# ClarkMcGrew/root-simple-mcmc

Measured on AMD Instinct MI355X. Metric: chain-steps/s on D=50 TDummyLogLikelihood, 65 536 chains; ESS/s + accept rate, higher is better.
Workload: dtype f64

## Files before the change

root-simple-mcmc_amd/csrc/smcmc_host.hpp:

```cpp
#pragma once

#include <hip/hip_runtime.h>

#include <cstddef>
#include <string>
#include <vector>

#include "smcmc.h"
#include "smcmc_event_sample_host.hpp"
#include "smcmc_kernels.hip.h"

namespace smcmc {

template <typename T, bool Pinned = false>
class Buffer {
public:
    Buffer() = default;
    ~Buffer() { release(); }
    Buffer(Buffer&& o) noexcept : p_(o.p_), n_(o.n_) { o.p_ = nullptr; o.n_ = 0; }
    Buffer& operator=(Buffer&& o) noexcept {
        if (this != &o) {
            release();
            p_ = o.p_; n_ = o.n_;
            o.p_ = nullptr; o.n_ = 0;
        }
        return *this;
    }
    Buffer(const Buffer&) = delete;
    Buffer& operator=(const Buffer&) = delete;

    hipError_t allocate(size_t n) {
        release();
        void* p = nullptr;
        const hipError_t e = Pinned ? hipHostMalloc(&p, n * sizeof(T), hipHostMallocDefault) : hipMalloc(&p, n * sizeof(T));
        if (e != hipSuccess) return e;
        p_ = static_cast<T*>(p);
        n_ = n;
        return hipSuccess;
    }
    size_t size() const { return n_; }
    T* get() const { return p_; }
    operator T*() const { return p_; }

private:
    void release() {
        if (p_) (void)(Pinned ? hipHostFree(p_) : hipFree(p_));
        p_ = nullptr;
        n_ = 0;
    }
    T* p_ = nullptr;
    size_t n_ = 0;
};
template <typename T> using DeviceBuffer = Buffer<T, false>;
template <typename T> using PinnedBuffer = Buffer<T, true>;

struct DeviceGuard {
    int prev = -1;
    bool switched = false;
    explicit DeviceGuard(int device) {
        if (hipGetDevice(&prev) == hipSuccess && prev != device) switched = (hipSetDevice(device) == hipSuccess);
    }
    ~DeviceGuard() {
        if (switched) (void)hipSetDevice(prev);
    }
    DeviceGuard(const DeviceGuard&) = delete;
    DeviceGuard& operator=(const DeviceGuard&) = delete;
};
#define ON_DEVICE(h) ::smcmc::DeviceGuard device_guard_((h)->device)

template <typename H>
int fail(H* h, int status, const std::string& msg) {
    if (h) h->error = msg;
    return status;
}

#define HIP_TRY(h, expr)                                                                                  \
    do {                                                                                                  \
        hipError_t e_ = (expr);                                                                           \
        if (e_ != hipSuccess)                                                                             \
            return ::smcmc::fail((h), SMCMC_ERR_HIP, std::string(#expr) + ": " + hipGetErrorString(e_)); \
    } while (0)

#define SMCMC_DP_ENTRY(n) n,
constexpr int kDPList[] = {SMCMC_FOR_EACH_DP(SMCMC_DP_ENTRY)};
#undef SMCMC_DP_ENTRY
constexpr int kNumDP = sizeof(kDPList) / sizeof(kDPList[0]);

inline bool event_likelihood(int like) {
    return like == SMCMC_LIKE_EVENT_SAMPLE || like == SMCMC_LIKE_EVENT_TEMPLATE || like == SMCMC_LIKE_EVENT_SHAPE;
}
inline int event_likelihood_dim(int like) { return like == SMCMC_LIKE_EVENT_SHAPE ? SMCMC_ESH_DIM : SMCMC_ES_DIM; }

inline bool stress_likelihood(int like) {
    return like == SMCMC_LIKE_ASYM || like == SMCMC_LIKE_HORRIFIC || like == SMCMC_LIKE_CONSTRAINED;
}

inline int pick_dp(int dim, int like) {
    for (int i = 0; i < kNumDP; ++i)
        if (dim <= kDPList[i] && (!stress_likelihood(like) || kDPList[i] == 31 || kDPList[i] == 63)) return kDPList[i];
    return -1;
}

template <typename T>
__global__ void fill_kernel(T* dst, size_t n, T v) {
    const size_t i = (size_t)blockIdx.x * blockDim.x + threadIdx.x;
    if (i < n) dst[i] = v;
}

template <typename T>
hipError_t fill(T* dst, size_t n, T v, hipStream_t stream) {
    const int threads = 256;
    hipLaunchKernelGGL(HIP_KERNEL_NAME(fill_kernel<T>), dim3((unsigned)((n + threads - 1) / threads)), dim3(threads), 0,
                       stream, dst, n, v);
    return hipGetLastError();
}

template <typename H>
int check_like_params(H* h, int like, size_t user_max, const char* user_rule, std::vector<double>& prm) {
    const std::vector<double>& p = h->like_params;
    prm.clear();
    switch (like) {
        case SMCMC_LIKE_QUADFORM:
            if (p.size() != (size_t)h->dim * h->dim)
                return fail(h, SMCMC_ERR_INVALID, "QUADFORM needs dim*dim likelihood parameters (the Error matrix)");
            break;
        case SMCMC_LIKE_ROSENBROCK:
            prm = {p.empty() ? 100.0 : p[0]};
            break;
        case SMCMC_LIKE_ASYM:
            if (p.empty()) prm = {-1.0, 100.0};
            else if (p.size() == 2) prm = p;
            else return fail(h, SMCMC_ERR_INVALID, "ASYM takes {positiveSlope, negativeSlope}");
            break;
        case SMCMC_LIKE_CONSTRAINED:
            if (p.size() != 2 + 2 * (size_t)h->dim)
                return fail(h, SMCMC_ERR_INVALID,
                            "CONSTRAINED needs {SummedValues, SummedConstraint, ExpectedValues[dim], PriorConstraints[dim]}");
            prm = p;
            break;
        case SMCMC_LIKE_EVENT_SAMPLE:
        case SMCMC_LIKE_EVENT_TEMPLATE:
        case SMCMC_LIKE_EVENT_SHAPE: {
            const char* why = es_check_like(like, p.data(), p.size());
            if (why) return fail(h, SMCMC_ERR_INVALID, why);
            break;
        }
        case SMCMC_LIKE_USER:
            if (p.size() > user_max) return fail(h, SMCMC_ERR_INVALID, user_rule);
            prm = p;
            break;
        default: break;
    }
    return SMCMC_OK;
}

// ... 2 lines not shown
```

root-simple-mcmc_amd/csrc/smcmc_inst.hip:

```cpp
#include "smcmc_kernels.hip.h"
#include "smcmc_vaat_kernel.hip.h"

#if !defined(SMCMC_DP) || !defined(SMCMC_LIKE)
#error "compile with -DSMCMC_DP=<padded dimension> -DSMCMC_LIKE=<likelihood id>"
#endif

namespace smcmc {

template <int DP, int LIKE, bool EXACT, bool FULLU, bool MOM, bool SPECIAL>
static hipError_t go(const StepParams& p, hipStream_t s) {
    if constexpr (LIKE == SMCMC_LIKE_EVENT_SAMPLE || LIKE == SMCMC_LIKE_EVENT_TEMPLATE || LIKE == SMCMC_LIKE_EVENT_SHAPE) {
        auto kernel = step_kernel<DP, LIKE, EXACT, FULLU, MOM, SPECIAL>;
        constexpr int cap = event_lds_bytes(LIKE, event_max_bins(LIKE));
        if (p.like_lds_bytes <= 0 || p.like_lds_bytes > cap) return hipErrorInvalidValue;
        if (LIKE != SMCMC_LIKE_EVENT_SAMPLE && !p.like_park) return hipErrorInvalidValue;
        const hipError_t e = hipFuncSetAttribute(reinterpret_cast<const void*>(kernel), hipFuncAttributeMaxDynamicSharedMemorySize, cap);
        if (e != hipSuccess) return e;
        hipLaunchKernelGGL(kernel, dim3(p.npad / kWave), dim3(kWave), (size_t)p.like_lds_bytes, s, p);
        return hipGetLastError();
    }
    hipLaunchKernelGGL(HIP_KERNEL_NAME(step_kernel<DP, LIKE, EXACT, FULLU, MOM, SPECIAL>), dim3(p.npad / kWave),
                       dim3(kWave), 0, s, p);
    return hipGetLastError();
}

template <>
hipError_t launch_step_like<SMCMC_DP, SMCMC_LIKE>(const StepParams& p, bool exact, bool fullu, bool mom, bool special,
                                                  hipStream_t s) {
    constexpr int DP = SMCMC_DP, LIKE = SMCMC_LIKE;
#if SMCMC_LIKE == 7 || SMCMC_LIKE == 8 || SMCMC_LIKE == 9
    if (!exact) return hipErrorNotSupported;
    if (special) {
        if (fullu) return mom ? go<DP, LIKE, true, true, true, true>(p, s) : go<DP, LIKE, true, true, false, true>(p, s);
        return mom ? go<DP, LIKE, true, false, true, true>(p, s) : go<DP, LIKE, true, false, false, true>(p, s);
    }
    if (fullu) return mom ? go<DP, LIKE, true, true, true, false>(p, s) : go<DP, LIKE, true, true, false, false>(p, s);
    return mom ? go<DP, LIKE, true, false, true, false>(p, s) : go<DP, LIKE, true, false, false, false>(p, s);
#else
    if (special) {
        if (!exact) return hipErrorNotSupported;
        if (fullu) return mom ? go<DP, LIKE, true, true, true, true>(p, s) : go<DP, LIKE, true, true, false, true>(p, s);
        return mom ? go<DP, LIKE, true, false, true, true>(p, s) : go<DP, LIKE, true, false, false, true>(p, s);
    }
    if (fullu) return mom ? go<DP, LIKE, true, true, true, false>(p, s) : go<DP, LIKE, true, true, false, false>(p, s);
    if (exact) return mom ? go<DP, LIKE, true, false, true, false>(p, s) : go<DP, LIKE, true, false, false, false>(p, s);
    return mom ? go<DP, LIKE, false, false, true, false>(p, s) : go<DP, LIKE, false, false, false, false>(p, s);
#endif
}

#if (SMCMC_LIKE != 3 || defined(SMCMC_USER_LIKELIHOOD)) && SMCMC_LIKE != 7 && SMCMC_LIKE != 8 && SMCMC_LIKE != 9
template <>
hipError_t launch_vaat_like<SMCMC_DP, SMCMC_LIKE>(const VaatParams& p, bool exact, hipStream_t s) {
    constexpr int DP = SMCMC_DP, LIKE = SMCMC_LIKE;
    if (p.record != nullptr) {
        if (exact) hipLaunchKernelGGL(HIP_KERNEL_NAME(vaat_step_kernel<DP, LIKE, true, true>), dim3(p.npad / kWave), dim3(kWave), 0, s, p);
        else hipLaunchKernelGGL(HIP_KERNEL_NAME(vaat_step_kernel<DP, LIKE, false, true>), dim3(p.npad / kWave), dim3(kWave), 0, s, p);
        return hipGetLastError();
    }
    if (exact) hipLaunchKernelGGL(HIP_KERNEL_NAME(vaat_step_kernel<DP, LIKE, true>), dim3(p.npad / kWave), dim3(kWave), 0, s, p);
    else hipLaunchKernelGGL(HIP_KERNEL_NAME(vaat_step_kernel<DP, LIKE, false>), dim3(p.npad / kWave), dim3(kWave), 0, s, p);
    return hipGetLastError();
}
#endif

#if SMCMC_LIKE == 0
template <>
hipError_t launch_reduce<SMCMC_DP>(double* gacc, int ngroups, int D, double* chunk_sums, double* moments,
                                   hipStream_t s) {
    const int npk = (D + 1) * (D + 2) / 2;
    const int nchunks = (ngroups + kReduceChunk - 1) / kReduceChunk;
    hipLaunchKernelGGL(HIP_KERNEL_NAME(reduce_chunks_kernel<SMCMC_DP>), dim3((npk + 63) / 64, nchunks), dim3(64), 0, s,
// ... 10 lines not shown
```

root-simple-mcmc_amd/csrc/smcmc_kernels.hip.h:

```cpp
#pragma once

#include <hip/hip_runtime.h>
#include <stdint.h>

#include <type_traits>

#include "smcmc.h"
#include "smcmc_detmath.h"
#include "smcmc_event_sample.h"
#include "smcmc_step_deal.h"

namespace smcmc {

#define SMCMC_FOR_EACH_DP(X) X(7) X(15) X(31) X(47) X(50) X(63)

#define SMCMC_DP_ENTRY(n) n,
constexpr int kDpMacroList[] = {SMCMC_FOR_EACH_DP(SMCMC_DP_ENTRY)};
#undef SMCMC_DP_ENTRY
constexpr bool dp_lists_agree() {
    if (sizeof(kDpMacroList) / sizeof(kDpMacroList[0]) != (size_t)kNumDpFamilies) return false;
    for (int f = 0; f < kNumDpFamilies; ++f)
        if (kDpMacroList[f] != kDpFamilies[f]) return false;
    return true;
}
static_assert(dp_lists_agree(), "kDpFamilies of smcmc_step_deal.h restates SMCMC_FOR_EACH_DP: keep the two alike");

constexpr int kWave = 64;

typedef double f64x4 __attribute__((ext_vector_type(4)));

typedef const __attribute__((address_space(4))) double* cptr_f64;
typedef const __attribute__((address_space(3))) double* lds_cptr_f64;
typedef double f64x2 __attribute__((ext_vector_type(2)));
typedef const __attribute__((address_space(3))) f64x2* lds_cptr_f64x2;
__device__ __forceinline__ cptr_f64 as_const(const double* p) {
#pragma clang diagnostic push
#pragma clang diagnostic ignored "-Wold-style-cast"
    return (cptr_f64)p;
#pragma clang diagnostic pop
}


struct NormalTables { f64x2 le, ae; };
template <int DP>
constexpr bool kAsmReads = DP >= 47;
template <bool ASM>
__device__ __forceinline__ NormalTables normal_tables_fetch(uint32_t w0, uint32_t w1, uint32_t lt_base, uint32_t at_base) {
    NormalTables t;
    const uint32_t la = lt_base + 16u * smcmc_normal_log_index(w0), aa = at_base + 16u * smcmc_normal_angle_index_halfcircle(w1);
    if constexpr (ASM) {
        asm volatile("ds_read_b128 %0, %1" : "=v"(t.le) : "v"(la));
        asm volatile("ds_read_b128 %0, %1" : "=v"(t.ae) : "v"(aa));
    } else {
        t.le = *(volatile lds_cptr_f64x2)(uintptr_t)la;
        t.ae = *(volatile lds_cptr_f64x2)(uintptr_t)aa;
    }
    return t;
}
template <int N, bool ASM>
__device__ __forceinline__ void normal_tables_ready(NormalTables& a, NormalTables& b) {
    if constexpr (ASM) asm volatile("s_waitcnt lgkmcnt(%4)" : "+v"(a.le), "+v"(a.ae), "+v"(b.le), "+v"(b.ae) : "n"(N));
}
template <int N, bool ASM>
__device__ __forceinline__ void normal_tables_ready(NormalTables& a) {
    if constexpr (ASM) asm volatile("s_waitcnt lgkmcnt(%2)" : "+v"(a.le), "+v"(a.ae) : "n"(N));
}
__device__ __forceinline__ void normal_pair_lds(uint32_t w0, uint32_t w1, const NormalTables& t, double* n0, double* n1) {
#ifdef SMCMC_NORMAL_TEXTBOOK
    (void)t;
    smcmc_normal_pair(w0, w1, n0, n1);
    return;
#endif
#define SMCMC_LT_LDS(k, c) (t.le[c])
#define SMCMC_AT_LDS(c) (t.ae[c])
    SMCMC_NORMAL_PAIR_BODY_HALFCIRCLE(SMCMC_LT_LDS, SMCMC_AT_LDS)
#undef SMCMC_LT_LDS
#undef SMCMC_AT_LDS
}

template <int I, int N, typename F>
__device__ __forceinline__ void static_for_impl(F& f) {
    if constexpr (I < N) {
        f(std::integral_constant<int, I>{});
        static_for_impl<I + 1, N>(f);
    }
}
template <int N, typename F>
__device__ __forceinline__ void static_for(F&& f) { static_for_impl<0, N>(f); }

template <int DP, bool FULLU, int i, int c, int k = 0>
__device__ __forceinline__ void load_piece(uint32_t ubase, f64x2 (&dst)[kPiece / 2]) {
    typedef ULayout<DP, FULLU> UL;
    if constexpr (k < kPiece / 2) {
        if constexpr (c + 2 * k < UL::DPE) {
            constexpr int off = (UL::off(i) + (c - UL::j0(i)) + 2 * k) * 8;
            if constexpr (kAsmReads<DP>) asm volatile("ds_read_b128 %0, %1 offset:%2" : "=v"(dst[k]) : "v"(ubase), "n"(off));
            else dst[k] = *(lds_cptr_f64x2)(uintptr_t)(ubase + (uint32_t)off);
        }
        load_piece<DP, FULLU, i, c, k + 1>(ubase, dst);
    }
}
template <int N, int M, bool ASM>
// ... 414 lines not shown
            const double pj = xq[XL::row(j)];
            if constexpr (EXACT) logl -= h * e * pj;
            else logl = SMCMC_FMA(-(h * e), pj, logl);
        }
    }
    return logl;
}

struct QuadCsr {
    const int32_t* rowptr;
    const int32_t* cols;
    const double* vals;
    const int32_t* rows;
};
constexpr int kQuadChunk = 8;
typedef const __attribute__((address_space(4))) int32_t* cptr_i32;
__device__ __forceinline__ cptr_i32 as_const(const int32_t* p) {
#pragma clang diagnostic push
#pragma clang diagnostic ignored "-Wold-style-cast"
    return (cptr_i32)p;
#pragma clang diagnostic pop
}
template <bool EXACT, typename Point>
__device__ __forceinline__ double quadform_csr(const Point& point, const QuadCsr& q, int D) {
    const cptr_i32 rw = as_const(q.rows), cl = as_const(q.cols);
    const cptr_f64 vl = as_const(q.vals);
    const int nnz = as_const(q.rowptr)[0];
    double logl = 0.0;
    for (int k0 = 0; k0 < nnz; k0 += kQuadChunk) {
        int ri[kQuadChunk], ci[kQuadChunk];
        double e[kQuadChunk], pi[kQuadChunk], pj[kQuadChunk];
#pragma unroll
        for (int u = 0; u < kQuadChunk; ++u) {
            ri[u] = rw[k0 + u];
            ci[u] = cl[k0 + u];
            e[u] = vl[k0 + u];
        }
#pragma unroll
        for (int u = 0; u < kQuadChunk; ++u) {
            pi[u] = point(ri[u]);
            pj[u] = point(ci[u]);
        }
#pragma unroll
        for (int u = 0; u < kQuadChunk; ++u) {
            const double h = 0.5 * pi[u];
            if constexpr (EXACT) logl -= h * e[u] * pj[u];
            else logl = SMCMC_FMA(-(h * e[u]), pj[u], logl);
        }
    }
    (void)D;
    return logl;
}

template <int DP, int LIKE, bool EXACT, bool FULLU, bool MOMENTS, bool SPECIAL>
__global__ void __launch_bounds__(kWave, 2) step_kernel(const StepParams p) {
    constexpr int T = Geo<DP>::T;
    constexpr int NT = Geo<DP>::NT;
    constexpr int NB = Geo<DP>::NB;
    typedef ULayout<DP, FULLU> UL;
    constexpr bool HEADLINE = EXACT && !FULLU && !SPECIAL && DP == 50 && LIKE == SMCMC_LIKE_ISO_GAUSS;
    constexpr bool PAIRS = HEADLINE;
    constexpr bool FIXED_AW = HEADLINE && MOMENTS && AcceptBlock<DP>::FIXED;
    typedef XLayout<DP, MOMENTS, PAIRS> XL;
    static_assert(!PAIRS || DP % 2 == 0, "a lane's 16-byte accesses cover whole row pairs of the point");
    constexpr bool ZROW = HEADLINE && MOMENTS;
    static_assert(!ZROW || XL::ZERO_ROW == DP + 1, "the ones row's partner is the zero row");
    __shared__ alignas(PAIRS ? 16 : 8) double xs[XL::DOUBLES];
    __shared__ __attribute__((aligned(16))) double us[UL::SIZE];
    __shared__ __attribute__((aligned(16))) double ntab[384];

    double* es_hist = nullptr;
    if constexpr (LIKE == SMCMC_LIKE_EVENT_SAMPLE || LIKE == SMCMC_LIKE_EVENT_TEMPLATE || LIKE == SMCMC_LIKE_EVENT_SHAPE) {
        extern __shared__ __attribute__((aligned(16))) double es_dynamic[];
        es_hist = es_dynamic;
    }
    (void)es_hist;

    const int lane = threadIdx.x;
    const int group = blockIdx.x;
    const int chain = group * kWave + lane;
    const bool active = chain < p.nchains;
    const int D = p.dim;
    const size_t NP = (size_t)p.npad;
    const uint32_t gid = p.chain_offset + (uint32_t)chain;
    const cptr_f64 c0 = as_const(p.c0);
    const cptr_f64 likep = as_const(p.like);
    double* const xcol = xs + XL::LANE * lane;
    auto load_point = [&](double (&dst)[DP]) {
#pragma unroll
        for (int q = 0; q < DP / 2; ++q) {
            const f64x2 v = *(const f64x2*)(xcol + XL::row(2 * q));
            dst[2 * q] = v[0];
            dst[2 * q + 1] = v[1];
        }
    };
    auto store_point = [&](const double (&src)[DP]) {
#pragma unroll
        for (int q = 0; q < DP / 2; ++q) {
            f64x2 v;
            v[0] = src[2 * q];
            v[1] = src[2 * q + 1];
            *(f64x2*)(xcol + XL::row(2 * q)) = v;
        }
    };
    (void)load_point;
    (void)store_point;

    if constexpr (PAIRS) {
        double xin[DP];
#pragma unroll
        for (int d = 0; d < DP; ++d) xin[d] = active ? p.x[(size_t)d * NP + chain] : c0[d];
        store_point(xin);
    } else {
#pragma unroll
        for (int d = 0; d < DP; ++d) xcol[XL::row(d)] = active ? p.x[(size_t)d * NP + chain] : c0[d];
    }

    double* lf = p.lane_f64 + chain;
    int32_t* li = p.lane_i32 + chain;
    double logl = lf[SMCMC_LANE_LOGL * NP];
    double sigma = lf[SMCMC_LANE_SIGMA * NP];
    double acc_rate = lf[SMCMC_LANE_ACCEPTANCE * NP];
    double acc_trials = lf[SMCMC_LANE_ACCEPTANCE_TRIALS * NP];
    double rigid = lf[SMCMC_LANE_RIGIDITY * NP];
    double last_value = lf[SMCMC_LANE_LAST_VALUE * NP];
    double last_x0 = lf[SMCMC_LANE_LAST_X0 * NP];
    double step_rms = lf[SMCMC_LANE_STEP_RMS * NP];
    double logl_prop = lf[SMCMC_LANE_LOGL_PROPOSED * NP];
    int trials = li[SMCMC_LANE_TRIALS * NP];
    int succ = li[SMCMC_LANE_SUCCESSES * NP];
    int next_update = li[SMCMC_LANE_NEXT_UPDATE * NP];
    int naccept = li[SMCMC_LANE_NACCEPT * NP];
    int rms_trials = li[SMCMC_LANE_STEP_RMS_TRIALS * NP];
    int last_accept = li[SMCMC_LANE_LAST_ACCEPT * NP];

#pragma unroll
    for (int i = 0; i < DP; ++i) {
        for (int k = lane; k < UL::len(i); k += kWave) {
            const int j = UL::j0(i) + k;
            us[UL::off(i) + k] = (j < DP) ? p.U[i * DP + j] : 0.0;
        }
    }

    for (int k = lane; k < 128; k += kWave) ntab[k] = smcmc_log_table_dev[k];
    for (int k = lane; k < 64; k += kWave) {
        const double c = smcmc_angle_table_dev[2 * k], sn = smcmc_angle_table_dev[2 * k + 1];
        ntab[128 + 2 * k] = c;
        ntab[128 + 2 * k + 1] = sn;
        ntab[128 + 128 + 2 * k] = -sn;
        ntab[128 + 128 + 2 * k + 1] = c;
    }
    const uint32_t ltab = (uint32_t)(uintptr_t)(lds_cptr_f64)ntab, atab = ltab + 128u * 8u;

    constexpr bool STRIP = MOMENTS && Geo<DP>::STRIP;
    constexpr int NT16 = Geo<DP>::NT16;
    f64x4 acc[MOMENTS ? NT16 : 1];
    double accs[STRIP ? T : 1];
    double c0r[MOMENTS ? T : 1];
    int xrow[MOMENTS ? T : 1];
    double c0s = 0.0;
    int xsrow = 0;
    if constexpr (MOMENTS) {
#pragma unroll
        for (int t = 0; t < NT16; ++t)
#pragma unroll
            for (int r = 0; r < 4; ++r)
                acc[t][r] = p.gacc[(((size_t)group * NT + t) * 4 + r) * kWave + lane];
        if constexpr (STRIP) {
#pragma unroll
            for (int t = 0; t < T; ++t) accs[t] = p.gacc[(((size_t)group * NT + NT16 + t) * 4) * kWave + lane];
            const int r = 16 * Geo<DP>::T16 + (lane & 3);
            c0s = (r < DP) ? p.c0[r] : 0.0;
            xsrow = XL::row((r <= DP) ? r : (ZROW ? XL::ZERO_ROW : DP)) + XL::LANE * (lane >> 4);
        }
        if constexpr (PAIRS) {
            static_assert(XL::HELD == DP + 2, "the ones row and its partner are one pair");
            f64x2 ones;
            ones[0] = active ? 1.0 : 0.0;
            ones[1] = 0.0;
            *(f64x2*)(xcol + XL::row(DP)) = ones;
        } else {
            xcol[XL::row(DP)] = active ? 1.0 : 0.0;
        }
#pragma unroll
        for (int t = 0; t < T; ++t) {
            const int r = 16 * t + (lane & 15);
            c0r[t] = (r < DP) ? p.c0[r] : 0.0;
            xrow[t] = XL::row((r <= DP) ? r : (ZROW ? XL::ZERO_ROW : DP)) + XL::LANE * (lane >> 4);
        }
    }
    __syncthreads();

    constexpr bool OPF = MOMENTS && T >= 3 && kAsmReads<DP> && DP <= 50 && !FULLU && !SPECIAL;
    constexpr int KQ = 4 * 8 * XL::LANE;
    double raw[OPF ? T : 1], raws = 0.0;
    uint32_t xaddr[OPF ? T : 1], xsaddr = 0;
    if constexpr (OPF) {
#pragma unroll
        for (int t = 0; t < T; ++t) xaddr[t] = (uint32_t)(uintptr_t)(lds_cptr_f64)(xs + xrow[t]);
        if constexpr (STRIP) xsaddr = (uint32_t)(uintptr_t)(lds_cptr_f64)(xs + xsrow);
    }

    double xp[DP];
    const uint32_t aw = smcmc_accept_word((uint32_t)D);
#ifdef SMCMC_STEP_PROFILE
// ... 70 lines not shown
            if (dense) logl_prop = loglike_quadform_lds<DP, EXACT, XL>(xcol, likep + p.zero * (s + 1));
        }
        else if constexpr (LIKE == SMCMC_LIKE_EVENT_SAMPLE) logl_prop = event_sample_loglike<DP>(xp, likep + p.zero * (s + 1), es_hist, lane);
        else if constexpr (LIKE == SMCMC_LIKE_EVENT_TEMPLATE)
            logl_prop = event_two_pass_loglike<DP, false>(xp, likep + p.zero * (s + 1), es_hist, lane, p.like_park + chain, NP);
        else if constexpr (LIKE == SMCMC_LIKE_EVENT_SHAPE)
            logl_prop = event_two_pass_loglike<DP, true>(xp, likep + p.zero * (s + 1), es_hist, lane, p.like_park + chain, NP);
        else if constexpr (!RMS_AHEAD) logl_prop = loglike<DP, LIKE, EXACT>(xp, likep + p.zero * (s + 1), D);
        if constexpr (!RMS_AHEAD) SMCMC_PROF_MARK(PROF_LIKE);
        bool take;
        if (p.metropolis == 2) {
            take = true;
        } else if (!__builtin_isfinite(logl_prop) || logl_prop < -0.999999E+30) {
            take = false;
        } else {
            const double delta = logl_prop - logl;
            take = true;
            if (delta < 0.0) {
                if (p.metropolis == 1) take = false;
                else {
                    const double trial = smcmc_log_pos(smcmc_u01(uword));
                    if (delta < trial) take = false;
                }
            }
        }
        take = take && active;
        last_accept = take ? 1 : 0;
        if (take) {
            logl = logl_prop;
            ++naccept;
        }
        SMCMC_PROF_MARK(PROF_TEST);
        if (take != SWAP) {
            if constexpr (PAIRS) store_point(xp);
            else {
#pragma unroll
                for (int d = 0; d < DP; ++d) xcol[XL::row(d)] = xp[d];
            }
        }
        SMCMC_PROF_MARK(PROF_COMMIT);
        if constexpr (BOUNDARY) x0 = take ? xp[0] : x0;
        if constexpr (MOMENTS && BOUNDARY) asm volatile("" ::: "memory");
        else if constexpr (MOMENTS) __syncthreads();
        SMCMC_PROF_MARK(PROF_ENDWAIT);
        if (p.save_x != nullptr && ((s + 1) % p.save_stride) == 0 && active) {
            const size_t slot = (size_t)((s + 1) / p.save_stride - 1);
#pragma unroll
            for (int d = 0; d < DP; ++d) p.save_x[(slot * (size_t)DP + (size_t)d) * NP + chain] = xcol[XL::row(d)];
            p.save_logl[slot * NP + chain] = logl;
        }
    };

    int s0 = 0;
    if (p.has_forced && p.nsteps > 0) {
#pragma unroll
        for (int d = 0; d < DP; ++d) xp[d] = p.forced[(size_t)d * NP + chain];
        smcmc_u32x4 blk = smcmc_draw_block(p.seed, gid, (uint64_t)(p.step0 + 1u), aw >> 2, SMCMC_STREAM_STEP);
        finish_step(0, smcmc_select_word(blk, aw & 3u));
        s0 = 1;
    }

    if (SPECIAL && p.scan_dim >= 0) {
        const uint32_t sd = (uint32_t)p.scan_dim;
#pragma nounroll
        for (int s = s0; s < p.nsteps; ++s) {
            const uint64_t step = (uint64_t)(p.step0 + (uint32_t)s + 1u);
            const smcmc_u32x4 sblk = smcmc_draw_block(p.seed, gid, step, sd >> 2, SMCMC_STREAM_STEP);
            double val;
            if (p.scan_uniform) {
                val = p.scan_a + (p.scan_b - p.scan_a) * smcmc_u01(smcmc_select_word(sblk, sd & 3u));
            } else {
                double nc, ns;
                smcmc_normal_pair(smcmc_select_word(sblk, sd & 2u), smcmc_select_word(sblk, (sd & 2u) + 1u), &nc, &ns);
                val = p.scan_a + p.scan_b * ((sd & 1u) ? ns : nc);
            }
#pragma unroll
            for (int d = 0; d < DP; ++d) xp[d] = ((uint32_t)d == sd) ? val : xcol[XL::row(d)];
            const smcmc_u32x4 ablk = smcmc_draw_block(p.seed, gid, step, aw >> 2, SMCMC_STREAM_STEP);
            finish_step(s, smcmc_select_word(ablk, aw & 3u));
        }
        s0 = p.nsteps;
    }

    for (int s = s0; s < p.nsteps; ++s) {
        const uint64_t step = (uint64_t)(p.step0 + (uint32_t)s + 1u);
        SMCMC_PROF_MARK(PROF_LOOP);
        SMCMC_PROF_MARK(PROF_STAMP);

        if constexpr (TOP_FREE && PAIRS) load_point(xp);
        else if constexpr (TOP_FREE) {
#pragma unroll
            for (int d = 0; d < DP; ++d) xp[d] = xcol[XL::row(d)];
        }

        ++trials;
        if constexpr (!BOUNDARY) x0 = xcol[XL::row(0)];
        const bool moved = (logl != last_value) || (x0 != last_x0);
        if (moved) ++succ;
        acc_rate *= acc_trials;
        if (moved) acc_rate = acc_rate + 1.0;
        acc_rate /= acc_trials + 1.0;
        acc_trials = dmin(p.acc_window, acc_trials + 1.0);
        if (rigid < 500.0 && rigid > 0.0) {
            if (__builtin_fabs(acc_rate - p.target) < p.asig) {
                rigid += 0.5 * rigid / p.acc_window;
                rigid = dmin(200.0, rigid);
            }
            if (__builtin_fabs(acc_rate - p.target) > 4.0 * p.asig) {
                rigid -= 1.618 * 0.5 * rigid / p.acc_window;
                rigid = dmax(2.0, rigid);
            }
        }
        if (rigid > 0 && rigid < 100.0) {
            sigma *= smcmc_pow_small(acc_rate / p.target,
                                     dmin(1.0 / 500.0, 1.0 / (rigid * p.acc_window)));
        }
        if constexpr (!MOMENTS) {
            if (p.per_lane_update && moved && (--next_update) < 1) {
                double up = 0.5 * succ;
                next_update = (int)(p.acc_window + p.max_up - p.max_up / (up + 1.0));
                if (p.acc_w >= 0.0) {
                    acc_trials = dmax(1.0, p.acc_w * acc_trials);
                    acc_trials = dmin(acc_trials, p.acc_wW);
                }
            }
        }
        last_value = logl;
        last_x0 = x0;
        SMCMC_PROF_MARK(PROF_A);

        if constexpr (OPF) {
            fetch_operands<T, 0, KQ>(xaddr, raw);
            if constexpr (STRIP) fetch_operand<0, KQ>(xsaddr, raws);
        }
        if constexpr (!TOP_FREE && PAIRS) load_point(xp);
        else if constexpr (!TOP_FREE) {
#pragma unroll
            for (int d = 0; d < DP; ++d) xp[d] = xcol[XL::row(d)];
        }
        uint32_t uword = 0;
        uint32_t up = (uint32_t)(uintptr_t)(lds_cptr_f64)us;
        asm volatile("" : "+v"(up));
        double ma[MOMENTS ? T : 1];
        double ms = 0.0;
        constexpr bool PIPE = kAsmReads<DP>;
        smcmc_u32x4 blks[2];
        NormalTables tabs[2][2];
        auto draw_and_fetch = [&](auto bn) {
            constexpr int b1 = decltype(bn)::value;
            blks[b1 & 1] = smcmc_draw_block(p.seed, gid, step, (uint32_t)b1, SMCMC_STREAM_STEP);
            tabs[b1 & 1][0] = normal_tables_fetch<kAsmReads<DP>>(blks[b1 & 1].v[0], blks[b1 & 1].v[1], ltab, atab);
            if constexpr (4 * b1 + 2 < DP)
                tabs[b1 & 1][1] = normal_tables_fetch<kAsmReads<DP>>(blks[b1 & 1].v[2], blks[b1 & 1].v[3], ltab, atab);
        };
        if constexpr (PIPE) draw_and_fetch(std::integral_constant<int, 0>{});
        SMCMC_PROF_MARK(PROF_TOP);
        static_for<NB>([&](auto bc) {
            constexpr int b = decltype(bc)::value;
            typedef UPieces<DP, FULLU, b> PC;
            f64x2 cur[kPiece / 2], nxt[kPiece / 2];

            if constexpr (!PIPE) draw_and_fetch(bc);
            smcmc_u32x4& blk = blks[b & 1];
            if constexpr (FIXED_AW) {
                if constexpr (b == AcceptBlock<DP>::BLOCK) uword = smcmc_select_word(blk, aw & 3u);
            } else if ((uint32_t)b == (aw >> 2)) uword = smcmc_select_word(blk, aw & 3u);
            NormalTables& t0 = tabs[b & 1][0];
            NormalTables& t1 = tabs[b & 1][1];
            {
                constexpr int i0 = PC::row(0), c0p = PC::col(0);
                load_piece<DP, FULLU, i0, c0p>(up, cur);
                if constexpr (4 * b + 2 < DP) normal_tables_ready<piece_reads<DP, FULLU, c0p>(), kAsmReads<DP>>(t0, t1);
                else normal_tables_ready<piece_reads<DP, FULLU, c0p>(), kAsmReads<DP>>(t0);
                if constexpr (DEAL) __builtin_amdgcn_sched_barrier(0);
            }
            double n[4];
            normal_pair_lds(blk.v[0], blk.v[1], t0, &n[0], &n[1]);
            if constexpr (4 * b + 2 < DP) normal_pair_lds(blk.v[2], blk.v[3], t1, &n[2], &n[3]);
            else { n[2] = 0.0; n[3] = 0.0; }
            double sr[4];
#pragma unroll
            for (int q = 0; q < 4; ++q) sr[q] = sigma * n[q];
            __builtin_amdgcn_sched_barrier(0);
            SMCMC_PROF_MARK(PROF_NORMALS);

            static_for<PC::COUNT>([&](auto rc) {
                constexpr int r = decltype(rc)::value;
                constexpr int i = PC::row(r), c = PC::col(r);
                constexpr int g = PC::first_global() + r;
                (void)g;
                if constexpr (r + 1 < PC::COUNT) {
                    constexpr int i1 = PC::row(r + 1), c1 = PC::col(r + 1);
                    load_piece<DP, FULLU, i1, c1>(up, nxt);
                    piece_ready<piece_reads<DP, FULLU, c1>(), piece_reads<DP, FULLU, c>(), kAsmReads<DP>>(cur);
                    SMCMC_PROF_PIECE(PROF_PIECE_DRAIN, g);
                } else {
                    piece_ready<0, piece_reads<DP, FULLU, c>(), kAsmReads<DP>>(cur);
                    SMCMC_PROF_PIECE(PROF_PIECE_DRAIN, g);
                    if constexpr (PIPE && b + 1 < NB) draw_and_fetch(std::integral_constant<int, b + 1>{});
                }
                const double srow = sr[i - 4 * b];
#pragma unroll
                for (int k = 0; k < kPiece; ++k) {
                    const int j = c + k;
                    if (j < DP && (FULLU || j >= i)) {
                        const double u = cur[k / 2][k & 1];
// ... 65 lines not shown
                                acc[tile] = __builtin_amdgcn_mfma_f64_16x16x4f64(ma[ti], ma[tj], acc[tile], 0, 0, 0);
                                asm volatile("" : "+a"(acc[tile]));
                            } else {
                                constexpr int t = tile - NT16;
                                accs[t] = __builtin_amdgcn_mfma_f64_4x4x4f64(ms, ma[t], accs[t], 0, 0, 0);
                                asm volatile("" : "+a"(accs[t]));
                            }
                            if constexpr (tile == 0 && OPF && kk + 1 < 16) {
                                static_assert(((long)(kk + 1) * NT * G) / NM > g, "operand prefetch needs a piece boundary");
                                fetch_operands<T, kk + 1, KQ>(xaddr, raw);
                                if constexpr (STRIP) fetch_operand<kk + 1, KQ>(xsaddr, raws);
                            }
                        });
                    }
                }
                SMCMC_PROF_PIECE(PROF_PIECE_MATRIX, g);
                __builtin_amdgcn_sched_barrier(0);
                if constexpr (r + 1 < PC::COUNT) {
#pragma unroll
                    for (int k = 0; k < kPiece / 2; ++k) cur[k] = nxt[k];
                }
            });
            SMCMC_PROF_MARK(PROF_PIECES);
        });
        if (!FIXED_AW && (aw >> 2) >= (uint32_t)NB) {
            smcmc_u32x4 blk = smcmc_draw_block(p.seed, gid, step, aw >> 2, SMCMC_STREAM_STEP);
            uword = smcmc_select_word(blk, aw & 3u);
        }
        if (SPECIAL && p.uniform_mask != 0) {
            const cptr_f64 ub = as_const(p.uniform);
            uint64_t m = p.uniform_mask;
#pragma nounroll
            while (m != 0) {
                const uint32_t ud = (uint32_t)__builtin_ctzll(m);
                m &= m - 1;
                const smcmc_u32x4 ublk = smcmc_draw_block(p.seed, gid, step, ud >> 2, SMCMC_STREAM_STEP);
                const double lo = ub[ud], hi = ub[DP + ud];
                const double val = lo + (hi - lo) * smcmc_u01(smcmc_select_word(ublk, ud & 3u));
#pragma unroll
                for (int d = 0; d < DP; ++d) xp[d] = ((uint32_t)d == ud) ? val : xp[d];
            }
        }
        SMCMC_PROF_MARK(PROF_TAIL);
        finish_step(s, uword);
    }

#ifdef SMCMC_STEP_PROFILE
    if (p.prof != nullptr) {
#pragma unroll
        for (int q = 0; q < kProfSlots; ++q) p.prof[((size_t)group * kProfSlots + q) * kWave + lane] += prof.slot[q];
    }
#endif
    if constexpr (MOMENTS) {
#pragma unroll
        for (int t = 0; t < NT16; ++t)
#pragma unroll
            for (int r = 0; r < 4; ++r)
                p.gacc[(((size_t)group * NT + t) * 4 + r) * kWave + lane] = acc[t][r];
        if constexpr (STRIP) {
#pragma unroll
            for (int t = 0; t < T; ++t) p.gacc[(((size_t)group * NT + NT16 + t) * 4) * kWave + lane] = accs[t];
        }
    }
    if (active) {
#pragma unroll
        for (int d = 0; d < DP; ++d) p.x[(size_t)d * NP + chain] = xcol[XL::row(d)];
        lf[SMCMC_LANE_LOGL * NP] = logl;
        lf[SMCMC_LANE_SIGMA * NP] = sigma;
        lf[SMCMC_LANE_ACCEPTANCE * NP] = acc_rate;
        lf[SMCMC_LANE_ACCEPTANCE_TRIALS * NP] = acc_trials;
        lf[SMCMC_LANE_RIGIDITY * NP] = rigid;
        lf[SMCMC_LANE_LAST_VALUE * NP] = last_value;
        lf[SMCMC_LANE_LAST_X0 * NP] = last_x0;
        lf[SMCMC_LANE_STEP_RMS * NP] = step_rms;
        lf[SMCMC_LANE_LOGL_PROPOSED * NP] = logl_prop;
        li[SMCMC_LANE_TRIALS * NP] = trials;
        li[SMCMC_LANE_SUCCESSES * NP] = succ;
        li[SMCMC_LANE_NEXT_UPDATE * NP] = next_update;
        li[SMCMC_LANE_NACCEPT * NP] = naccept;
        li[SMCMC_LANE_STEP_RMS_TRIALS * NP] = rms_trials;
        li[SMCMC_LANE_LAST_ACCEPT * NP] = last_accept;
    }
}

constexpr int kReduceChunk = 32;

template <int DP>
__device__ __forceinline__ size_t packed_to_tile_offset(int k, int D) {
    int i = (int)((__builtin_sqrt(8.0 * (double)k + 1.0) - 1.0) * 0.5);
    while ((i + 1) * (i + 2) / 2 <= k) ++i;
    while (i * (i + 1) / 2 > k) --i;
    const int j = k - i * (i + 1) / 2;
    const int ri = (i == D) ? DP : i, rj = (j == D) ? DP : j;
    const int ti = ri >> 4, tj = rj >> 4, ii = ri & 15, jj = rj & 15;
    const int reg = ii >> 2;
    const int lane = jj + 16 * (ii & 3);
    return ((size_t)(ti * (ti + 1) / 2 + tj) * 4 + reg) * kWave + lane;
}

template <int DP>
__global__ void reduce_chunks_kernel(double* __restrict__ gacc, int ngroups, int D, double* __restrict__ chunk_sums) {
    constexpr int NT = Geo<DP>::NT;
    const int npk = (D + 1) * (D + 2) / 2;
    const int k = blockIdx.x * blockDim.x + threadIdx.x;
    const int chunk = blockIdx.y;
    if (k >= npk) return;
    const size_t off = packed_to_tile_offset<DP>(k, D);
    const size_t gstride = (size_t)NT * 4 * kWave;
    const int g0 = chunk * kReduceChunk;
    const int g1 = (g0 + kReduceChunk < ngroups) ? g0 + kReduceChunk : ngroups;
    double v[kReduceChunk];
#pragma unroll
    for (int q = 0; q < kReduceChunk; ++q) v[q] = (g0 + q < g1) ? gacc[(size_t)(g0 + q) * gstride + off] : 0.0;
#pragma unroll
// ... 65 lines not shown
```

root-simple-mcmc_amd/csrc/smcmc_step_deal.h:

```cpp
#pragma once

namespace smcmc {

constexpr int kPiece = 16;

template <int DP>
struct Geo {
    static constexpr int T = (DP + 1 + 15) / 16;
    static constexpr int NT = T * (T + 1) / 2;
    static constexpr int NB = (DP + 3) / 4;
    static constexpr int ROWS_MOMENTS = DP + 1;
    static constexpr bool STRIP = ((DP + 1) % 16 != 0) && ((DP + 1) % 16 <= 4);
    static constexpr int T16 = STRIP ? T - 1 : T;
    static constexpr int NT16 = T16 * (T16 + 1) / 2;
};

constexpr int kDpFamilies[] = {7, 15, 31, 47, 50, 63};
constexpr int kNumDpFamilies = sizeof(kDpFamilies) / sizeof(kDpFamilies[0]);

constexpr unsigned accept_word_of(unsigned dim) { return 2u * ((dim + 1u) / 2u); }

template <int DP>
struct AcceptBlock {
    static constexpr int lowest() {
        int prev = 0;
        for (int f = 0; f < kNumDpFamilies; ++f) {
            if (kDpFamilies[f] == DP) return prev + 1;
            prev = kDpFamilies[f];
        }
        return 1;
    }
    static constexpr int LOWEST = lowest();
    static constexpr int BLOCK = (int)(accept_word_of((unsigned)DP) >> 2);
    static constexpr bool fixed() {
        for (int d = LOWEST; d <= DP; ++d)
            if ((int)(accept_word_of((unsigned)d) >> 2) != BLOCK) return false;
        return BLOCK < Geo<DP>::NB;
    }
    static constexpr bool FIXED = fixed();
};

constexpr int kXStride = 66;
template <int DP, bool MOMENTS, bool PAIRS>
struct XLayout {
    static constexpr int ROWS = MOMENTS ? Geo<DP>::ROWS_MOMENTS : DP;
    static constexpr int PAIR_STRIDE = 64 * 16 + 32;
    static constexpr int HELD = PAIRS ? (ROWS + 1) / 2 * 2 : ROWS;
    static constexpr int LANE = PAIRS ? 2 : 1;
    static constexpr int DOUBLES = PAIRS ? HELD / 2 * (PAIR_STRIDE / 8) : ROWS * kXStride;
    static constexpr int BYTES = DOUBLES * 8;
    static constexpr int row(int r) { return PAIRS ? (r >> 1) * (PAIR_STRIDE / 8) + (r & 1) : r * kXStride; }
    static constexpr int offset(int r, int c) { return 8 * (row(r) + LANE * c); }
    static constexpr int ZERO_ROW = (PAIRS && MOMENTS && HELD > ROWS) ? ROWS : -1;
};

template <int DP, bool FULLU>
struct ULayout {
    static constexpr int DPE = DP + (DP & 1);
    static constexpr int j0(int i) { return FULLU ? 0 : (i & ~1); }
    static constexpr int len(int i) { return DPE - j0(i); }
    static constexpr int off(int i) {
        return FULLU ? i * DPE
                     : i * DPE - ((i & 1) ? 2 * (i / 2) * (i / 2) : 2 * (i / 2) * (i / 2 - 1));
    }
    static constexpr int SIZE = off(DP);
};

template <int DP, bool FULLU, int B>
struct UPieces {
    typedef ULayout<DP, FULLU> UL;
    static constexpr int rows() { return (4 * B + 4 <= DP) ? 4 : (DP - 4 * B); }
    static constexpr int per_row(int i) { return (UL::len(i) + kPiece - 1) / kPiece; }
    static constexpr int count() {
        int n = 0;
        for (int q = 0; q < rows(); ++q) n += per_row(4 * B + q);
        return n;
    }
    static constexpr int COUNT = count();
    static constexpr int first_global() {
        int n = 0;
        for (int i = 0; i < 4 * B; ++i) n += per_row(i);
        return n;
    }
    static constexpr int row(int r) {
        int i = 4 * B;
        while (r >= per_row(i)) { r -= per_row(i); ++i; }
        return i;
    }
    static constexpr int col(int r) {
        int i = 4 * B;
        while (r >= per_row(i)) { r -= per_row(i); ++i; }
        return UL::j0(i) + r * kPiece;
    }
};

template <int DP, bool FULLU, int c>
constexpr int piece_reads() {
    int n = 0;
    for (int k = 0; k < kPiece / 2; ++k) n += (c + 2 * k < ULayout<DP, FULLU>::DPE) ? 1 : 0;
    return n;
}

constexpr int tile_row(int tile) {
    int ti = 0;
    while ((ti + 1) * (ti + 2) / 2 <= tile) ++ti;
    return ti;
}

template <int DP>
struct StepDeal {
    typedef ULayout<DP, false> UL;
    static constexpr int NQ = 16;
    static constexpr int T = Geo<DP>::T;
    static constexpr int NT = Geo<DP>::NT;
    static constexpr int NT16 = Geo<DP>::STRIP ? Geo<DP>::NT16 : NT;
    static constexpr int NS = NT - NT16;
    static constexpr int NM = NQ * NT;
    static constexpr int PREFETCH = T + (NS > 0 ? 1 : 0);
// ... 169 lines not shown
```

Baseline: 4.449 billion.

## Share U matrix and replicated normal tables across four-wave workgroups in headline step kernel

```diff
diff --git a/root-simple-mcmc_amd/csrc/smcmc_host.hpp b/root-simple-mcmc_amd/csrc/smcmc_host.hpp
--- a/root-simple-mcmc_amd/csrc/smcmc_host.hpp
+++ b/root-simple-mcmc_amd/csrc/smcmc_host.hpp
@@ -2,6 +2,7 @@
 
 #include <hip/hip_runtime.h>
 
+#include <atomic>
 #include <cstddef>
 #include <string>
 #include <vector>
@@ -101,6 +102,20 @@
     return -1;
 }
 
+template <typename Site>
+hipError_t raise_dynamic_lds_once(const void* kernel, int bytes) {
+    constexpr int kMaxDevices = 64;
+    static std::atomic<bool> done[kMaxDevices];
+    int device = 0;
+    hipError_t e = hipGetDevice(&device);
+    if (e != hipSuccess) return e;
+    const bool tracked = device >= 0 && device < kMaxDevices;
+    if (tracked && done[device].load(std::memory_order_acquire)) return hipSuccess;
+    e = hipFuncSetAttribute(kernel, hipFuncAttributeMaxDynamicSharedMemorySize, bytes);
+    if (e == hipSuccess && tracked) done[device].store(true, std::memory_order_release);
+    return e;
+}
+
 template <typename T>
 __global__ void fill_kernel(T* dst, size_t n, T v) {
     const size_t i = (size_t)blockIdx.x * blockDim.x + threadIdx.x;
diff --git a/root-simple-mcmc_amd/csrc/smcmc_inst.hip b/root-simple-mcmc_amd/csrc/smcmc_inst.hip
--- a/root-simple-mcmc_amd/csrc/smcmc_inst.hip
+++ b/root-simple-mcmc_amd/csrc/smcmc_inst.hip
@@ -1,3 +1,6 @@
+#include <utility>
+
+#include "smcmc_host.hpp"
 #include "smcmc_kernels.hip.h"
 #include "smcmc_vaat_kernel.hip.h"
 
@@ -17,6 +20,14 @@
         const hipError_t e = hipFuncSetAttribute(reinterpret_cast<const void*>(kernel), hipFuncAttributeMaxDynamicSharedMemorySize, cap);
         if (e != hipSuccess) return e;
         hipLaunchKernelGGL(kernel, dim3(p.npad / kWave), dim3(kWave), (size_t)p.like_lds_bytes, s, p);
+        return hipGetLastError();
+    }
+    if constexpr (kStepHeadline<DP, LIKE, EXACT, FULLU, SPECIAL>) {
+        auto kernel = step_kernel<DP, LIKE, EXACT, FULLU, MOM, SPECIAL>;
+        constexpr int lds = StepWorkgroupLds<DP, MOM>::TOTAL;
+        const hipError_t e = raise_dynamic_lds_once<std::integer_sequence<int, DP, LIKE, EXACT, FULLU, MOM, SPECIAL>>(reinterpret_cast<const void*>(kernel), lds);
+        if (e != hipSuccess) return e;
+        hipLaunchKernelGGL(kernel, dim3(step_blocks_for(p.npad / kWave)), dim3(kStepWaves * kWave), (size_t)lds, s, p);
         return hipGetLastError();
     }
     hipLaunchKernelGGL(HIP_KERNEL_NAME(step_kernel<DP, LIKE, EXACT, FULLU, MOM, SPECIAL>), dim3(p.npad / kWave),
diff --git a/root-simple-mcmc_amd/csrc/smcmc_kernels.hip.h b/root-simple-mcmc_amd/csrc/smcmc_kernels.hip.h
--- a/root-simple-mcmc_amd/csrc/smcmc_kernels.hip.h
+++ b/root-simple-mcmc_amd/csrc/smcmc_kernels.hip.h
@@ -44,10 +44,10 @@
 struct NormalTables { f64x2 le, ae; };
 template <int DP>
 constexpr bool kAsmReads = DP >= 47;
-template <bool ASM>
+template <bool ASM, int LSH = 4, int ASH = 4>
 __device__ __forceinline__ NormalTables normal_tables_fetch(uint32_t w0, uint32_t w1, uint32_t lt_base, uint32_t at_base) {
     NormalTables t;
-    const uint32_t la = lt_base + 16u * smcmc_normal_log_index(w0), aa = at_base + 16u * smcmc_normal_angle_index_halfcircle(w1);
+    const uint32_t la = lt_base + (smcmc_normal_log_index(w0) << LSH), aa = at_base + (smcmc_normal_angle_index_halfcircle(w1) << ASH);
     if constexpr (ASM) {
         asm volatile("ds_read_b128 %0, %1" : "=v"(t.le) : "v"(la));
         asm volatile("ds_read_b128 %0, %1" : "=v"(t.ae) : "v"(aa));
@@ -568,22 +568,41 @@
     return logl;
 }
 
+template <int DP, int LIKE, bool EXACT, bool FULLU, bool SPECIAL>
+constexpr bool kStepHeadline = EXACT && !FULLU && !SPECIAL && DP == 50 && LIKE == SMCMC_LIKE_ISO_GAUSS;
+
 template <int DP, int LIKE, bool EXACT, bool FULLU, bool MOMENTS, bool SPECIAL>
-__global__ void __launch_bounds__(kWave, 2) step_kernel(const StepParams p) {
+__global__ void __launch_bounds__((kStepHeadline<DP, LIKE, EXACT, FULLU, SPECIAL> ? kStepWaves * kWave : kWave),
+                                  (kStepHeadline<DP, LIKE, EXACT, FULLU, SPECIAL> ? 1 : 2)) step_kernel(const StepParams p) {
     constexpr int T = Geo<DP>::T;
     constexpr int NT = Geo<DP>::NT;
     constexpr int NB = Geo<DP>::NB;
     typedef ULayout<DP, FULLU> UL;
-    constexpr bool HEADLINE = EXACT && !FULLU && !SPECIAL && DP == 50 && LIKE == SMCMC_LIKE_ISO_GAUSS;
+    constexpr bool HEADLINE = kStepHeadline<DP, LIKE, EXACT, FULLU, SPECIAL>;
     constexpr bool PAIRS = HEADLINE;
     constexpr bool FIXED_AW = HEADLINE && MOMENTS && AcceptBlock<DP>::FIXED;
     typedef XLayout<DP, MOMENTS, PAIRS> XL;
     static_assert(!PAIRS || DP % 2 == 0, "a lane's 16-byte accesses cover whole row pairs of the point");
     constexpr bool ZROW = HEADLINE && MOMENTS;
     static_assert(!ZROW || XL::ZERO_ROW == DP + 1, "the ones row's partner is the zero row");
-    __shared__ alignas(PAIRS ? 16 : 8) double xs[XL::DOUBLES];
-    __shared__ __attribute__((aligned(16))) double us[UL::SIZE];
-    __shared__ __attribute__((aligned(16))) double ntab[384];
+    constexpr bool SHARED = HEADLINE;
+    typedef StepWorkgroupLds<DP, MOMENTS> WL;
+    static_assert(!SHARED || (PAIRS && WL::FITS && WL::IMAGE_BYTES == XL::BYTES), "the wavefronts' images lie end to end, within the CU's LDS");
+    __shared__ alignas(PAIRS ? 16 : 8) double xs_own[SHARED ? 2 : XL::DOUBLES];
+    __shared__ __attribute__((aligned(16))) double us_own[SHARED ? 2 : UL::SIZE];
+    __shared__ __attribute__((aligned(16))) double ntab_own[SHARED ? 2 : 384];
+    constexpr int NTHREADS = SHARED ? kStepWaves * kWave : kWave;
+    int wave = 0;
+    if constexpr (SHARED) wave = __builtin_amdgcn_readfirstlane((int)(threadIdx.x >> 6));
+    double* xs = xs_own;
+    double* us = us_own;
+    double* ntab = ntab_own;
+    if constexpr (SHARED) {
+        extern __shared__ __attribute__((aligned(16))) double wg_lds[];
+        xs = wg_lds + (WL::IMAGE_BYTES / 8) * wave;
+        us = wg_lds + WL::US / 8;
+        ntab = wg_lds + WL::LOG / 8;
+    }
 
     double* es_hist = nullptr;
     if constexpr (LIKE == SMCMC_LIKE_EVENT_SAMPLE || LIKE == SMCMC_LIKE_EVENT_TEMPLATE || LIKE == SMCMC_LIKE_EVENT_SHAPE) {
@@ -592,10 +611,13 @@
     }
     (void)es_hist;
 
-    const int lane = threadIdx.x;
-    const int group = blockIdx.x;
+    const int lane = SHARED ? (int)(threadIdx.x & (kWave - 1)) : (int)threadIdx.x;
+    const int ngroups = p.npad / kWave;
+    const bool live = !SHARED || step_group_of((int)blockIdx.x, wave) < ngroups;
+    const int group = !SHARED ? (int)blockIdx.x : live ? step_group_of((int)blockIdx.x, wave) : ngroups - 1;
+    const int nsteps = live ? p.nsteps : 0;
     const int chain = group * kWave + lane;
-    const bool active = chain < p.nchains;
+    const bool active = live && chain < p.nchains;
     const int D = p.dim;
     const size_t NP = (size_t)p.npad;
     const uint32_t gid = p.chain_offset + (uint32_t)chain;
@@ -650,23 +672,50 @@
     int rms_trials = li[SMCMC_LANE_STEP_RMS_TRIALS * NP];
     int last_accept = li[SMCMC_LANE_LAST_ACCEPT * NP];
 
+    const int tid = (int)threadIdx.x;
 #pragma unroll
     for (int i = 0; i < DP; ++i) {
-        for (int k = lane; k < UL::len(i); k += kWave) {
+        for (int k = tid; k < UL::len(i); k += NTHREADS) {
             const int j = UL::j0(i) + k;
             us[UL::off(i) + k] = (j < DP) ? p.U[i * DP + j] : 0.0;
         }
     }
 
-    for (int k = lane; k < 128; k += kWave) ntab[k] = smcmc_log_table_dev[k];
-    for (int k = lane; k < 64; k += kWave) {
-        const double c = smcmc_angle_table_dev[2 * k], sn = smcmc_angle_table_dev[2 * k + 1];
-        ntab[128 + 2 * k] = c;
-        ntab[128 + 2 * k + 1] = sn;
-        ntab[128 + 128 + 2 * k] = -sn;
-        ntab[128 + 128 + 2 * k + 1] = c;
-    }
-    const uint32_t ltab = (uint32_t)(uintptr_t)(lds_cptr_f64)ntab, atab = ltab + 128u * 8u;
+    uint32_t ltab, atab;
+    if constexpr (SHARED) {
+        typedef LogTableLayout LT;
+        typedef AngleTableLayout AT;
+        double* const atb = ntab + (WL::ANGLE - WL::LOG) / 8;
+        for (int s = tid; s < LT::SLOTS; s += NTHREADS) {
+            const int k = LT::slot_entry(s);
+            f64x2 v;
+            v[0] = smcmc_log_table_dev[2 * k];
+            v[1] = smcmc_log_table_dev[2 * k + 1];
+            *(f64x2*)(ntab + LT::slot_offset(s) / 8) = v;
+        }
+        for (int s = tid; s < AT::SLOTS; s += NTHREADS) {
+            const int e = AT::slot_entry(s), k = e & 63;
+            const double c = smcmc_angle_table_dev[2 * k], sn = smcmc_angle_table_dev[2 * k + 1];
+            f64x2 v;
+            v[0] = (e < 64) ? c : -sn;
+            v[1] = (e < 64) ? sn : c;
+            *(f64x2*)(atb + AT::slot_offset(s) / 8) = v;
+        }
+        ltab = (uint32_t)(uintptr_t)(lds_cptr_f64)ntab + (uint32_t)LT::lane_offset(lane);
+        atab = (uint32_t)(uintptr_t)(lds_cptr_f64)atb + (uint32_t)AT::lane_offset(lane);
+    } else {
+        for (int k = lane; k < 128; k += kWave) ntab[k] = smcmc_log_table_dev[k];
+        for (int k = lane; k < 64; k += kWave) {
+            const double c = smcmc_angle_table_dev[2 * k], sn = smcmc_angle_table_dev[2 * k + 1];
+            ntab[128 + 2 * k] = c;
+            ntab[128 + 2 * k + 1] = sn;
+            ntab[128 + 128 + 2 * k] = -sn;
+            ntab[128 + 128 + 2 * k + 1] = c;
+        }
+        ltab = (uint32_t)(uintptr_t)(lds_cptr_f64)ntab;
+        atab = ltab + 128u * 8u;
+    }
+    constexpr int LSH = SHARED ? LogTableLayout::SHIFT : 4, ASH = SHARED ? AngleTableLayout::SHIFT : 4;
 
     constexpr bool STRIP = MOMENTS && Geo<DP>::STRIP;
     constexpr int NT16 = Geo<DP>::NT16;
@@ -843,7 +892,7 @@
     };
 
     int s0 = 0;
-    if (p.has_forced && p.nsteps > 0) {
+    if (p.has_forced && nsteps > 0) {
 #pragma unroll
         for (int d = 0; d < DP; ++d) xp[d] = p.forced[(size_t)d * NP + chain];
         smcmc_u32x4 blk = smcmc_draw_block(p.seed, gid, (uint64_t)(p.step0 + 1u), aw >> 2, SMCMC_STREAM_STEP);
@@ -854,7 +903,7 @@
     if (SPECIAL && p.scan_dim >= 0) {
         const uint32_t sd = (uint32_t)p.scan_dim;
 #pragma nounroll
-        for (int s = s0; s < p.nsteps; ++s) {
+        for (int s = s0; s < nsteps; ++s) {
             const uint64_t step = (uint64_t)(p.step0 + (uint32_t)s + 1u);
             const smcmc_u32x4 sblk = smcmc_draw_block(p.seed, gid, step, sd >> 2, SMCMC_STREAM_STEP);
             double val;
@@ -870,10 +919,10 @@
             const smcmc_u32x4 ablk = smcmc_draw_block(p.seed, gid, step, aw >> 2, SMCMC_STREAM_STEP);
             finish_step(s, smcmc_select_word(ablk, aw & 3u));
         }
-        s0 = p.nsteps;
-    }
-
-    for (int s = s0; s < p.nsteps; ++s) {
+        s0 = nsteps;
+    }
+
+    for (int s = s0; s < nsteps; ++s) {
         const uint64_t step = (uint64_t)(p.step0 + (uint32_t)s + 1u);
         SMCMC_PROF_MARK(PROF_LOOP);
         SMCMC_PROF_MARK(PROF_STAMP);
@@ -940,9 +989,9 @@
         auto draw_and_fetch = [&](auto bn) {
             constexpr int b1 = decltype(bn)::value;
             blks[b1 & 1] = smcmc_draw_block(p.seed, gid, step, (uint32_t)b1, SMCMC_STREAM_STEP);
-            tabs[b1 & 1][0] = normal_tables_fetch<kAsmReads<DP>>(blks[b1 & 1].v[0], blks[b1 & 1].v[1], ltab, atab);
+            tabs[b1 & 1][0] = normal_tables_fetch<kAsmReads<DP>, LSH, ASH>(blks[b1 & 1].v[0], blks[b1 & 1].v[1], ltab, atab);
             if constexpr (4 * b1 + 2 < DP)
-                tabs[b1 & 1][1] = normal_tables_fetch<kAsmReads<DP>>(blks[b1 & 1].v[2], blks[b1 & 1].v[3], ltab, atab);
+                tabs[b1 & 1][1] = normal_tables_fetch<kAsmReads<DP>, LSH, ASH>(blks[b1 & 1].v[2], blks[b1 & 1].v[3], ltab, atab);
         };
         if constexpr (PIPE) draw_and_fetch(std::integral_constant<int, 0>{});
         SMCMC_PROF_MARK(PROF_TOP);
@@ -1114,14 +1163,16 @@
     }
 #endif
     if constexpr (MOMENTS) {
-#pragma unroll
-        for (int t = 0; t < NT16; ++t)
-#pragma unroll
-            for (int r = 0; r < 4; ++r)
-                p.gacc[(((size_t)group * NT + t) * 4 + r) * kWave + lane] = acc[t][r];
-        if constexpr (STRIP) {
-#pragma unroll
-            for (int t = 0; t < T; ++t) p.gacc[(((size_t)group * NT + NT16 + t) * 4) * kWave + lane] = accs[t];
+        if (live) {
+#pragma unroll
+            for (int t = 0; t < NT16; ++t)
+#pragma unroll
+                for (int r = 0; r < 4; ++r)
+                    p.gacc[(((size_t)group * NT + t) * 4 + r) * kWave + lane] = acc[t][r];
+            if constexpr (STRIP) {
+#pragma unroll
+                for (int t = 0; t < T; ++t) p.gacc[(((size_t)group * NT + NT16 + t) * 4) * kWave + lane] = accs[t];
+            }
         }
     }
     if (active) {
diff --git a/root-simple-mcmc_amd/csrc/smcmc_step_deal.h b/root-simple-mcmc_amd/csrc/smcmc_step_deal.h
--- a/root-simple-mcmc_amd/csrc/smcmc_step_deal.h
+++ b/root-simple-mcmc_amd/csrc/smcmc_step_deal.h
@@ -54,6 +54,35 @@
     static constexpr int ZERO_ROW = (PAIRS && MOMENTS && HELD > ROWS) ? ROWS : -1;
 };
 
+template <int ENTRIES, int COPIES>
+struct NormalTableLayout {
+    static_assert(COPIES >= 1 && COPIES <= 16 && (COPIES & (COPIES - 1)) == 0, "a power of two, at most one per bank quad");
+    static constexpr int ENTRY_BYTES = 16;
+    static constexpr int STRIDE = ENTRY_BYTES * COPIES;
+    static constexpr int SLOTS = ENTRIES * COPIES;
+    static constexpr int BYTES = SLOTS * ENTRY_BYTES;
+    static constexpr int shift() {
+        int s = 0;
+        while ((1 << s) < STRIDE) ++s;
+        return s;
+    }
+    static constexpr int SHIFT = shift();
+    static constexpr int copy_of(int lane) { return lane & (COPIES - 1); }
+    static constexpr int lane_offset(int lane) { return ENTRY_BYTES * copy_of(lane); }
+    static constexpr int offset(int copy, int k) { return k * STRIDE + ENTRY_BYTES * copy; }
+    static constexpr int slot_offset(int s) { return ENTRY_BYTES * s; }
+    static constexpr int slot_entry(int s) { return s / COPIES; }
+};
+
+#ifndef SMCMC_NTAB_LOG_COPIES
+#define SMCMC_NTAB_LOG_COPIES 8
+#endif
+#ifndef SMCMC_NTAB_ANGLE_COPIES
+#define SMCMC_NTAB_ANGLE_COPIES 16
+#endif
+typedef NormalTableLayout<64, SMCMC_NTAB_LOG_COPIES> LogTableLayout;
+typedef NormalTableLayout<128, SMCMC_NTAB_ANGLE_COPIES> AngleTableLayout;
+
 template <int DP, bool FULLU>
 struct ULayout {
     static constexpr int DPE = DP + (DP & 1);
@@ -64,6 +93,24 @@
                      : i * DPE - ((i & 1) ? 2 * (i / 2) * (i / 2) : 2 * (i / 2) * (i / 2 - 1));
     }
     static constexpr int SIZE = off(DP);
+};
+
+constexpr int kStepWaves = 4;
+constexpr int kLdsPerCU = 160 * 1024;
+constexpr int step_group_of(int block, int wave) { return kStepWaves * block + wave; }
+constexpr int step_blocks_for(int groups) { return (groups + kStepWaves - 1) / kStepWaves; }
+template <int DP, bool MOMENTS>
+struct StepWorkgroupLds {
+    typedef XLayout<DP, MOMENTS, true> XL;
+    static constexpr int round16(int n) { return (n + 15) / 16 * 16; }
+    static constexpr int IMAGE_BYTES = round16(XL::BYTES);
+    static constexpr int image(int wave) { return wave * IMAGE_BYTES; }
+    static constexpr int US = kStepWaves * IMAGE_BYTES;
+    static constexpr int US_BYTES = round16(8 * ULayout<DP, false>::SIZE);
+    static constexpr int LOG = US + US_BYTES;
+    static constexpr int ANGLE = LOG + LogTableLayout::BYTES;
+    static constexpr int TOTAL = ANGLE + AngleTableLayout::BYTES;
+    static constexpr bool FITS = TOTAL <= kLdsPerCU;
 };
 
 template <int DP, bool FULLU, int B>
```

Result: faster. 4.506 billion, median of 6 (+1.3%).
